# edwinb-ai/MolecularDynamics.jl

Hardware: AMD Instinct MI355X
Metric: particle-steps/sec + achieved HBM GB/s, 1M LJ particles rho=0.897, 1/2/4/8 GPUs (higher is better)
Workload: dtype f64; 1 GPU; BASELINE configs[2]: N=1048576 monodisperse LJ 3D rho=0.897 r_cut=2.5 dt=0.001 NVT Bussi tau=0.1 kT=1.4737, per GPU; particles_per_gpu=1048576, parallelism=1 GPU, step_loop=fused (k_step_tile: one launch per step + k_finalize), global_particles=1048576, tiled_force_kernel=True, max_tile_halo=2081, energies_every_step=False, thermo_frequency=2589

## Files before the change

include/mdhip.h:

```cpp
#ifndef MDHIP_H
#define MDHIP_H

#include <stdint.h>

#ifdef __cplusplus
extern "C" {
#endif

typedef struct md_ctx md_ctx;

enum { MD_POT_LJ = 0, MD_POT_PSEUDOHS = 1, MD_POT_POLYDISPERSE = 2, MD_POT_LJ_MODIFIED = 3, MD_POT_CUSTOM = 100 };

enum { MD_NVE = 0, MD_NVT = 1 };

int md_create(int dim, int64_t n_particles, const double *box, double list_cutoff, int device_id, md_ctx **out);
int md_destroy(md_ctx *ctx);

const char *md_last_error(md_ctx *ctx);

int md_set_potential(md_ctx *ctx, int kind, const double *params, int nparams);

int md_set_potential_source(md_ctx *ctx, const char *hip_src, const char *entry_name, const double *params,
                            int nparams);

// ... 65 lines not shown
                  const double *q, int nq);
int md_cage_origin(md_ctx *ctx, int slot);
int md_cage_sample(md_ctx *ctx, const int32_t *slots, const int32_t *rows, int count);
int md_cage_particles(md_ctx *ctx, int32_t *nnb, double *d2cr, int32_t *broken);
int md_cage_read(md_ctx *ctx, int64_t *nsamples, double *sums, int64_t *counts, int64_t *hist_broken, int64_t *overflow);
int md_cage_reset(md_ctx *ctx);

int md_kinetic(md_ctx *ctx, double *kinetic);

int md_scale_velocities(md_ctx *ctx, double s);

typedef struct {
    int64_t steps;
    int64_t rebuilds;
    int64_t violations;
    int64_t n_ghost;
    int64_t max_neighbors;
    double avg_neighbors;
    int64_t force_launches;
    double force_ms;
    int64_t max_halo;
    int64_t tiled;
    int64_t prunes;
    int64_t kickdrift_launches;
    double kickdrift_ms;
    int64_t fused;
    int64_t walked_outer;
    int64_t walked_inner;
    int64_t prune_launches_timed;
    double prune_ms;
    int64_t rebuilds_timed;
    double rebuild_ms;
    int64_t fused_build;
} md_stats;
int md_profile(md_ctx *ctx, int enable);
int md_get_stats(md_ctx *ctx, md_stats *out);

int md_create_domain(int dim, int64_t n_global, int64_t n_cap, const double *box, double list_cutoff,
                     int device_id, int rank, int nranks, md_ctx **out);
int md_dom_set_uniform(md_ctx *ctx, int uniform, double sigma);
int md_dom_upload(md_ctx *ctx, int64_t n_own, const int32_t *ids, const double *x, const double *v, const double *f,
                  const int32_t *images, const double *diameters);
int md_dom_download(md_ctx *ctx, int64_t cap, int64_t *n_own, int32_t *ids, double *x, double *v, double *f,
                    int32_t *images);
int md_dom_migrate_pack(md_ctx *ctx, int64_t *nsend );
int md_dom_migrate_unpack(md_ctx *ctx, const int64_t *nrecv );
int md_dom_halo_pack(md_ctx *ctx, int64_t *nsend );
int md_dom_halo_unpack(md_ctx *ctx, const int64_t *nrecv );
int md_dom_build(md_ctx *ctx);
int md_dom_set_step_buffers(md_ctx *ctx, void *send_left, void *send_right, void *recv_left, void *recv_right,
                            int64_t capacity_doubles);
int md_dom_get_sendbuf(md_ctx *ctx, int side, int64_t ndoubles, void *dst, int dst_is_device);
int md_dom_put_recvbuf(md_ctx *ctx, int side, int64_t ndoubles, const void *src, int src_is_device);
int md_dom_step_begin(md_ctx *ctx, double dt, int *violated);
int md_dom_step_end(md_ctx *ctx, double dt, int want_uw, double *uwk);
int md_dom_forces(md_ctx *ctx, double dt, int kick, int want_uw, double *uwk);
int md_dom_set_scale(md_ctx *ctx, double scale);
int md_dom_counts(md_ctx *ctx, int64_t *out );

int md_set_stream(md_ctx *ctx, void *hip_stream);
int md_dom_async_begin(md_ctx *ctx, int64_t nsteps, double dt, int ensemble, double tau, double nf, const double *ktemp,
                       const double *r1, const double *r2, int64_t prune_interval, void *flag_dev ,
                       void *kuw_dev );
int md_dom_step_a(md_ctx *ctx, double dt, int step);
int md_dom_step_b(md_ctx *ctx, double dt, int step, int want_uw);
int md_dom_step_c(md_ctx *ctx, int step, int want_uw);
// ... 19 lines not shown
```

moleculardynamics/jl_amd/_lib.py:

```python
import ctypes as C
import os

_HERE = os.path.dirname(os.path.abspath(__file__))
SO_PATH = os.path.join(_HERE, "csrc", "libmdhip.so")

MD_POT_LJ, MD_POT_PSEUDOHS, MD_POT_POLYDISPERSE, MD_POT_LJ_MODIFIED, MD_POT_CUSTOM = 0, 1, 2, 3, 100
MD_NVE, MD_NVT = 0, 1
MD_CLUSTER_ALL, MD_CLUSTER_SOLID = 0, 1

EXPORTS = [
    "md_create", "md_destroy", "md_last_error", "md_set_potential", "md_set_potential_source", "md_set_skin",
    "md_set_inner_skin",
    "md_upload", "md_download", "md_snapshot_begin", "md_snapshot_end", "md_compute_forces", "md_neighbor_pairs", "md_run", "md_kinetic",
    "md_scale_velocities", "md_profile", "md_get_stats", "md_version", "md_fire_minimize", "md_run_brownian",
    "md_create_domain", "md_dom_set_uniform", "md_dom_upload", "md_dom_download", "md_dom_migrate_pack",
    "md_dom_migrate_unpack", "md_dom_halo_pack", "md_dom_halo_unpack", "md_dom_build", "md_dom_get_sendbuf",
    "md_dom_put_recvbuf", "md_dom_set_step_buffers", "md_dom_step_begin", "md_dom_step_end", "md_dom_forces", "md_dom_set_scale",
    "md_dom_counts", "md_set_stream", "md_dom_async_begin", "md_dom_step_a", "md_dom_step_b", "md_dom_step_c",
    "md_dom_async_end", "md_dom_comm_unique_id", "md_dom_comm_init", "md_dom_run_window", "md_dom_rebuild",
    "md_dom_enable_pruning", "md_dom_max_disp0", "md_dom_invalidate_inner",
    "md_rdf_setup", "md_rdf_sample", "md_rdf_read", "md_rdf_reset",
    "md_dyn_setup", "md_dyn_origin", "md_dyn_sample", "md_dyn_read", "md_dyn_reset",
    "md_sq_setup", "md_sq_sample", "md_sq_rho", "md_sq_read", "md_sq_reset",
    "md_stress_setup", "md_stress_sample", "md_stress_tensor", "md_stress_read", "md_stress_reset",
    "md_boo_setup", "md_boo_sample", "md_boo_particles", "md_boo_qlm", "md_boo_read", "md_boo_reset",
    "md_cluster_setup", "md_cluster_sample", "md_cluster_particles", "md_cluster_read", "md_cluster_reset",
    "md_cage_setup", "md_cage_origin", "md_cage_sample", "md_cage_particles", "md_cage_read", "md_cage_reset",
]


class MdStats(C.Structure):
    _fields_ = [("steps", C.c_int64), ("rebuilds", C.c_int64), ("violations", C.c_int64), ("n_ghost", C.c_int64),
                ("max_neighbors", C.c_int64), ("avg_neighbors", C.c_double), ("force_launches", C.c_int64),
                ("force_ms", C.c_double), ("max_halo", C.c_int64), ("tiled", C.c_int64), ("prunes", C.c_int64),
                ("kickdrift_launches", C.c_int64), ("kickdrift_ms", C.c_double), ("fused", C.c_int64),
                ("walked_outer", C.c_int64), ("walked_inner", C.c_int64), ("prune_launches_timed", C.c_int64),
                ("prune_ms", C.c_double), ("rebuilds_timed", C.c_int64), ("rebuild_ms", C.c_double),
                ("fused_build", C.c_int64)]


class MdhipError(RuntimeError):
    pass


_lib = None


def load():
    global _lib
    if _lib is not None:
        return _lib
    if not os.path.exists(SO_PATH):
        raise MdhipError(
            f"{SO_PATH} not found: build it with `python -c 'import __graft_entry__ as g; g.build()'` or "
            "`make -C moleculardynamics/jl_amd/csrc`. There is no CPU fallback.")
    L = C.CDLL(SO_PATH)
    vp, dp, ip = C.c_void_p, C.POINTER(C.c_double), C.POINTER(C.c_int32)
    L.md_create.argtypes = [C.c_int, C.c_int64, dp, C.c_double, C.c_int, C.POINTER(vp)]
    L.md_create.restype = C.c_int
    L.md_destroy.argtypes = [vp]
    L.md_destroy.restype = C.c_int
    L.md_last_error.argtypes = [vp]
    L.md_last_error.restype = C.c_char_p
    L.md_set_potential.argtypes = [vp, C.c_int, dp, C.c_int]
    L.md_set_potential.restype = C.c_int
    L.md_set_potential_source.argtypes = [vp, C.c_char_p, C.c_char_p, dp, C.c_int]
    L.md_set_potential_source.restype = C.c_int
    L.md_set_skin.argtypes = [vp, C.c_double]
    L.md_set_skin.restype = C.c_int
    L.md_set_inner_skin.argtypes = [vp, C.c_double]
    L.md_set_inner_skin.restype = C.c_int
# ... 141 lines not shown
```

moleculardynamics/jl_amd/csrc/md_build_tile.hpp:

```cpp
#pragma once

#define MD_BT_THREADS 512
#define MD_SCAP 3584
#define MD_NCMAX 1024
#define MD_NEMAX 36
#define MD_INF_CELL 0x7fffffff
#define MD_SWB 8

#define MD_HALF_CELLS 14

typedef float md_f2 __attribute__((ext_vector_type(2)));

template <int D>
__device__ __forceinline__ unsigned tile_sweep_word(md_f2 xi2, md_f2 yi2, md_f2 zi2, md_f2 rl2, int qa, int qb,
                                                    const float *px, const float *py, const float *pz)
{
    unsigned w = ~0u;
    for (int q0 = qa; q0 < qb; q0 += 4) {
        float4 x4 = *(const float4 *)(px + q0);
        float4 y4 = *(const float4 *)(py + q0);
        md_f2 dxa = md_f2{x4.x, x4.y} - xi2, dxb = md_f2{x4.z, x4.w} - xi2;
        md_f2 dya = md_f2{y4.x, y4.y} - yi2, dyb = md_f2{y4.z, y4.w} - yi2;
        md_f2 da = dxa * dxa, db = dxb * dxb;
        da = __builtin_elementwise_fma(dya, dya, da);
        db = __builtin_elementwise_fma(dyb, dyb, db);
        if constexpr (D == 3) {
            float4 z4 = *(const float4 *)(pz + q0);
            md_f2 dza = md_f2{z4.x, z4.y} - zi2, dzb = md_f2{z4.z, z4.w} - zi2;
            da = __builtin_elementwise_fma(dza, dza, da);
            db = __builtin_elementwise_fma(dzb, dzb, db);
        }
        const md_f2 ta = rl2 - da, tb = rl2 - db;
        w = __builtin_amdgcn_alignbit(w, __float_as_uint(ta.x), 31);
        w = __builtin_amdgcn_alignbit(w, __float_as_uint(ta.y), 31);
        w = __builtin_amdgcn_alignbit(w, __float_as_uint(tb.x), 31);
        w = __builtin_amdgcn_alignbit(w, __float_as_uint(tb.y), 31);
// ... 14 lines not shown
        mask0[ci] = 0u;
        mask1[ci] = 0u;
        qstart[ci] = 0;
        int nbi = n0 + ci;
        if (nbi >= n1) continue;
        int lo = ctab_row[nbi];
        if (lo == 0xffff) continue;
        int qs = coff[lo], qe = coff[lo + 1];
        if (qe - qs > 64) {
            *too_big = true;
            continue;
        }
        qstart[ci] = qs;
        unsigned m0 = tile_sweep_word<D>(xi2, yi2, zi2, rl2, qs, min(qs + 32, qe), px, py, pz);
        unsigned m1 = tile_sweep_word<D>(xi2, yi2, zi2, rl2, qs + 32, qe, px, py, pz);
        const unsigned so = (unsigned)(self_q - qs);
        if (so < (unsigned)(qe - qs)) {
            if (so < 32u)
                m0 &= ~(1u << so);
            else
                m1 &= ~(1u << (so - 32u));
        }
        if (m0) atomicOr(&refmask[2 * lo], m0);
        if (m1) atomicOr(&refmask[2 * lo + 1], m1);
        mask0[ci] = m0;
        mask1[ci] = m1;
        cnt += __popc(m0) + __popc(m1);
    }
    return cnt;
}

#define MD_BBMAX 1024
#define MD_ROWPITCH 132
#define MD_BT_POOL 68864

template <bool GUARD>
__device__ __forceinline__ int tile_emit_word(unsigned m, int qb, const uint16_t *newidx, uint16_t *row,
                                              uint16_t *grow, int lane, int maxn, int cnt, int rs)
{
    while (m) {
        const int b1 = __ffs((int)m) - 1;
        const unsigned m1 = m & (m - 1u);
        const int b2 = __ffs((int)m1) - 1;
        m = m1 & (m1 - 1u);
        if (!GUARD || cnt + 1 < MD_ROWPITCH) {
            row[cnt] = (uint16_t)(qb + b1);
            if (m1) row[cnt + 1] = (uint16_t)(qb + b2);
        } else {
            if (cnt < MD_ROWPITCH)
                row[cnt] = (uint16_t)(qb + b1);
            else if (cnt < maxn)
                grow[row_off(cnt, lane)] = (uint16_t)((unsigned)newidx[qb + b1] * (unsigned)rs);
            if (m1 && cnt + 1 < maxn) grow[row_off(cnt + 1, lane)] = (uint16_t)((unsigned)newidx[qb + b2] * (unsigned)rs);
        }
        cnt += m1 ? 2 : 1;
    }
    return cnt;
}

template <bool GUARD>
__device__ __forceinline__ int tile_sweep_emit_lds(const unsigned *mask0, const unsigned *mask1, const int *qstart,
                                                   const uint16_t *newidx, uint16_t *row, uint16_t *grow, int lane,
                                                   int maxn, int cnt0, int rs)
{
    int cnt = cnt0;
#pragma unroll
    for (int ci = 0; ci < MD_HALF_CELLS; ++ci) {
        const int qs = qstart[ci];
        cnt = tile_emit_word<GUARD>(mask0[ci], qs, newidx, row, grow, lane, maxn, cnt, rs);
        cnt = tile_emit_word<GUARD>(mask1[ci], qs + 32, newidx, row, grow, lane, maxn, cnt, rs);
    }
    return cnt;
}


template <bool GUARD>
__device__ __forceinline__ int tile_compact_word(unsigned m, int base, int src0, uint16_t *newidx, uint32_t *hrow,
                                                 int hcap, int run)
{
    while (m) {
        const int bit = __ffs((int)m) - 1;
        m &= m - 1u;
        newidx[base + bit] = (uint16_t)run;
        if (!GUARD || run < hcap) hrow[run] = (uint32_t)(src0 + bit);
        ++run;
    }
    return run;
}

__device__ __forceinline__ float tile_staged_coord(float v) { return fabsf(v) < 1.0e29f ? v : 1.0e30f; }
__device__ __forceinline__ float tile_own_coord(float v) { return fabsf(v) < 1.0e29f ? v : -1.0e30f; }

template <int D>
__global__ void __launch_bounds__(MD_BT_THREADS)
    k_build_tile(int n, DevState s, BoxGrid g, float rl2f, const int32_t *__restrict__ cell_start,
                 const int32_t *__restrict__ cell_end, uint16_t *__restrict__ nlist16, int maxn,
                 int32_t *__restrict__ nneigh, int32_t *__restrict__ nmax_tile, uint32_t *__restrict__ halo, int hcap,
                 int32_t *__restrict__ halo_count, Scalars *sc, long long *__restrict__ stamps, int rs)
{
#define MD_STAMP(i)                                                                                   \
    do {                                                                                              \
        if (stamps && threadIdx.x == 0) stamps[(size_t)blockIdx.x * 10 + (i)] = (long long)clock64(); \
    } while (0)
    MD_STAMP(0);
    __shared__ __attribute__((aligned(16))) unsigned char pool[MD_BT_POOL];
    float *px = (float *)pool, *py = px + MD_SCAP, *pz = py + MD_SCAP;
    unsigned *refmask = (unsigned *)(pool + 43008);
    int *ucell = (int *)(pool + 51200);
    int *coff = (int *)(pool + 55296);
    int *lcell = (int *)(pool + 59408);
    uint16_t *ctab = (uint16_t *)(pool + 63504);
    uint16_t *lmap = (uint16_t *)(pool + 65552);
    uint16_t *blk2u = (uint16_t *)(pool + 67600);
    unsigned char *ccnt = (unsigned char *)(pool + 67840);
    __shared__ uint16_t newidx[MD_SCAP];
    __shared__ int cntA[MD_TILE], cntB[MD_TILE];
    __shared__ int sh_misc[16];
    __shared__ int sh_scan[16];
    __shared__ int sh_ne[MD_NEMAX];
    __shared__ int sh_ne_e[MD_NEMAX][3];

    const int tile = blockIdx.x;
    const int tid = threadIdx.x, lane = tid & 63;
    const int half = tid / MD_TILE;
    const int pt = tid - half * MD_TILE;
    const int k = tile * MD_TILE + pt;
    const bool active = k < n;
    const double4 *__restrict__ P = s.pos;
    const int NNB = (D == 3) ? 27 : 9;
    const int nA = (NNB + 1) / 2;

    const double4 org = P[tile * MD_TILE];
    double4 pd = P[active ? k : n - 1];
    const float xi = tile_own_coord((float)(pd.x - org.x)), yi = tile_own_coord((float)(pd.y - org.y)),
                zi = (D == 3) ? tile_own_coord((float)(pd.z - org.z)) : 0.f;
    int ec[3];
    cell_coords<D>(pd, g, ec);
#pragma unroll
    for (int c = 0; c < D; ++c) ec[c] += 1;
    const int mycell = ext_linear(ec, g);
    if (tid == 0) sh_misc[0] = mycell;
    const int last_active = min(n - 1, tile * MD_TILE + MD_TILE - 1) - tile * MD_TILE;
    if (tid == last_active) sh_misc[1] = mycell;
    if (tid == 0) {
        sh_misc[2] = 0;
        sh_misc[4] = sh_misc[5] = sh_misc[6] = 0x7fffffff;
        sh_misc[7] = sh_misc[8] = sh_misc[9] = -1;
// ... 120 lines not shown
    }
    int self_q = -1;
    if (active) {
        int uc = ctab[myci * NNB + (NNB >> 1)];
        self_q = coff[uc] + (k - cell_start[mycell]);
    }
    __syncthreads();
    MD_STAMP(4);
    const int wt = tile * (MD_TILE / 64) + (pt >> 6);
    const int n0 = half ? nA : 0, n1 = half ? NNB : nA;
    unsigned hmask0[MD_HALF_CELLS], hmask1[MD_HALF_CELLS];
    int qstart[MD_HALF_CELLS];
    int cnt = 0;
    bool too_big = false;
    if (active)
        cnt = tile_sweep_mark<D>(xi, yi, zi, ctab + myci * NNB, rl2f, self_q, n0, n1, px, py, pz, coff, refmask, hmask0,
                                 hmask1, qstart, &too_big);
    else {
#pragma unroll
        for (int ci = 0; ci < MD_HALF_CELLS; ++ci) {
            hmask0[ci] = hmask1[ci] = 0u;
            qstart[ci] = 0;
        }
    }
    if (too_big) atomicOr(&sc->halo_overflow, 4);
    if (half == 0)
        cntA[pt] = cnt;
    else
        cntB[pt] = cnt;
    __syncthreads();
    MD_STAMP(5);
    int H;
    {
        const int per = (MD_NCMAX + MD_BT_THREADS - 1) / MD_BT_THREADS;
        int c = 0;
        for (int q = 0; q < per; ++q) {
            int u = tid * per + q;
            if (u < nu) c += __popc(refmask[2 * u]) + __popc(refmask[2 * u + 1]);
        }
        int run = block_excl_scan(c, sh_scan, &H);
        uint32_t *hrow = halo + (size_t)tile * hcap;
        for (int q = 0; q < per; ++q) {
            int u = tid * per + q;
            if (u >= nu) continue;
            const int base = coff[u], src0 = cell_start[ucell[u]];
            const unsigned r0 = refmask[2 * u], r1 = refmask[2 * u + 1];
            if (run + __popc(r0) + __popc(r1) <= hcap) {
                run = tile_compact_word<false>(r0, base, src0, newidx, hrow, hcap, run);
                run = tile_compact_word<false>(r1, base + 32, src0 + 32, newidx, hrow, hcap, run);
            } else {
                run = tile_compact_word<true>(r0, base, src0, newidx, hrow, hcap, run);
                run = tile_compact_word<true>(r1, base + 32, src0 + 32, newidx, hrow, hcap, run);
            }
        }
        if (tid == 0) {
            halo_count[tile] = H;
            atomicMax(&sc->hmax, H);
            if (H > hcap || (H + 1) * rs > 65535) atomicOr(&sc->halo_overflow, 1);
        }
    }
    const int totp = cntA[pt] + cntB[pt];
    if (half == 0) {
        int tot = active ? totp : 0;
        if (active) {
            nneigh[k] = tot;
            if (tot > maxn) {
                atomicOr(&sc->overflow, 1);
                tot = maxn;
            }
        }
        int m = wave_max_i(tot);
        m = (m + 3) & ~3;
        if (m > maxn) m = maxn;
        if (lane == 0) {
            nmax_tile[wt] = m;
            sh_misc[10 + (pt >> 6)] = m;
        }
    }
    MD_STAMP(6);
// ... 49 lines not shown
```

moleculardynamics/jl_amd/csrc/md_kernels.hpp:

```cpp
#ifndef MD_RTC
#pragma once
#include <hip/hip_runtime.h>
#include <stdint.h>
#else
typedef __hip_internal::uint64_t uint64_t;
typedef __hip_internal::uint32_t uint32_t;
typedef __hip_internal::int32_t int32_t;
typedef __hip_internal::uint16_t uint16_t;
#endif

#define MD_BLOCK 256
#define MD_WAVE 64
#define MD_SENTINEL_POS 1.0e100
#define MD_VAL_SRC_BITS 26
#define MD_VAL_SRC_MASK ((1u << MD_VAL_SRC_BITS) - 1u)
#define MD_NO_VIOLATION 0x7fffffff

enum { POT_LJ = 0, POT_PSEUDOHS = 1, POT_POLYDISPERSE = 2, POT_LJ_MOD = 3, POT_CUSTOM = 100 };

struct DevState {
    double4 *pos;
    double *v[3];
    double *f[3];
    int32_t *img[3];
// ... 1231 lines not shown
    if constexpr (KICK) {
        double t = block_sum(ke, red);
        if (threadIdx.x == 0) partials[bid] = t;
    }
    if constexpr (WANT_UW) {
        double tu = block_sum(us, red);
        double tw = block_sum(ws, red);
        if (threadIdx.x == 0) {
            partials[nblk_total + bid] = tu;
            partials[2 * nblk_total + bid] = tw;
        }
    }
    MD_SSTAMP(5);
#undef MD_SSTAMP
}

struct StepBufs {
    const double2 *recA;
    double2 *recB;
    size_t rstride;
    const double *fA[3];
    double *fB[3];
    double4 *posB;
};

template <int D, int POT, bool UNIFORM, bool WANT_UW, bool PRUNE>
__global__ void __launch_bounds__(MD_TILE)
    k_step_tile(int n, DevState s, StepBufs sb, PotParams pp, const uint16_t *__restrict__ nlist16, int maxn,
                const int32_t *__restrict__ nmax_tile, const uint32_t *__restrict__ halo, int hcap,
                const int32_t *__restrict__ halo_count, double dt, double skin_half, double inner_half, int use_d1,
                double *__restrict__ partials, int nblk_total, Scalars *__restrict__ sc, int step,
                uint16_t *__restrict__ rows_in, int32_t *__restrict__ nmax_in, double rin2,
                long long *__restrict__ stamps, uint32_t *__restrict__ halo_in, int hcap_in,
                int32_t *__restrict__ halo_in_count, const int32_t *__restrict__ tile_list = nullptr)
{
#define MD_SSTAMP(i)                                                                                   \
    do {                                                                                               \
        if (stamps && (threadIdx.x & 63) == 0)                                                         \
            stamps[((size_t)blockIdx.x * 4 + (threadIdx.x >> 6)) * 8 + (i)] = (long long)clock64();   \
    } while (0)
    constexpr int RS = UNIFORM ? 24 : 32;
    extern __shared__ __attribute__((aligned(16))) unsigned char smem[];
    __shared__ double red[16];
    if (sc->first_viol < step) return;
    MD_SSTAMP(0);
    int bid = xcd_remap(blockIdx.x, gridDim.x);
    if (tile_list) bid = tile_list[bid];
    int H = halo_count[bid];
    const uint32_t *hl = halo + (size_t)bid * hcap;
    int k = bid * MD_TILE + threadIdx.x;
    bool active = k < n;
    int kk = active ? k : n - 1;
    int lane = threadIdx.x & 63;
    int wt = bid * (MD_TILE / 64) + (threadIdx.x >> 6);
    const ushort4 *row4 = (const ushort4 *)(nlist16 + ((size_t)wt * maxn) * 64) + lane;
    PruneRow rin64;
    rin64.base = PRUNE ? (unsigned char *)(rows_in + ((size_t)__builtin_amdgcn_readfirstlane(wt) * maxn) * 64) : nullptr;
    rin64.off = (unsigned)lane * 8u;
    unsigned long long acc = 0ull;
    int cin = 0;
    int m = nmax_tile[wt];
    const double alpha = sc->scale;
    const double adt = alpha * dt;
    const double2 *RA0 = sb.recA, *RA1 = RA0 + sb.rstride, *RA2 = RA1 + sb.rstride, *RA3 = RA2 + sb.rstride;
    double2 a0 = RA0[kk], a1 = RA1[kk], a2 = RA2[kk];
    double sig_own = pp.sig_u;
    if constexpr (!UNIFORM) sig_own = RA3[kk].x;
    double fprev[3] = {0.0, 0.0, 0.0}, xr[3] = {0.0, 0.0, 0.0};
#pragma unroll
    for (int c = 0; c < D; ++c) {
        fprev[c] = sb.fA[c][kk];
        xr[c] = PRUNE ? s.x0[c][kk] : s.x1[c][kk];
    }
    constexpr int G = MD_UNROLL / 4;
    ushort4 jn[G];
#pragma unroll
    for (int g = 0; g < G; ++g) jn[g] = row4[(size_t)((4 * g < m) ? g : 0) * 64];
    MD_SSTAMP(1);
#ifndef MD_STAGE_NB
#define MD_STAGE_NB ((!PRUNE && UNIFORM && !WANT_UW) ? 6 : 8)
#endif
    constexpr int NB = MD_STAGE_NB;
    for (int h0 = 0; h0 <= H; h0 += NB * MD_TILE) {
        uint32_t idx[NB];
#pragma unroll
        for (int i = 0; i < NB; ++i) {
            int h = h0 + i * MD_TILE + threadIdx.x;
            idx[i] = (h < H) ? hl[h] : 0xffffffffu;
        }
        double2 r0[NB], r1[NB], r2[NB], r3[NB];
#pragma unroll
        for (int i = 0; i < NB; ++i) {
            bool ok = idx[i] != 0xffffffffu;
            size_t j = ok ? (size_t)(idx[i] & 0x3ffffffu) : 0;
            r0[i] = RA0[j];
            r1[i] = RA1[j];
            r2[i] = RA2[j];
            if constexpr (!UNIFORM) r3[i] = RA3[j];
        }
#pragma unroll
        for (int i = 0; i < NB; ++i) {
            int h = h0 + i * MD_TILE + threadIdx.x;
            bool ok = idx[i] != 0xffffffffu;
            double x = __builtin_fma(adt, r1[i].y, r0[i].x);
            double y = __builtin_fma(adt, r2[i].x, r0[i].y);
            double z = (D == 3) ? __builtin_fma(adt, r2[i].y, r1[i].x) : 0.0;
            uint32_t code = ok ? (idx[i] >> 26) : 0u;
            if (code) shift_xyz(x, y, z, code, s.boxL, s.tric, s.cellA);
            if (!ok) {
                x = MD_SENTINEL_POS;
                y = MD_SENTINEL_POS;
                z = (D == 3) ? MD_SENTINEL_POS : 0.0;
            }
            if (h <= H) {
                double *rec = (double *)(smem + (size_t)h * RS);
                rec[0] = x;
                rec[1] = y;
                rec[2] = z;
                if constexpr (!UNIFORM) rec[3] = ok ? r3[i].x : 1.0;
            }
        }
    }
    const double pown[3] = {a0.x, a0.y, a1.x}, vown[3] = {a1.y, a2.x, a2.y};
    double vh[3] = {0.0, 0.0, 0.0}, xn[3] = {0.0, 0.0, 0.0};
    double disp2 = 0.0;
#pragma unroll
    for (int c = 0; c < D; ++c) {
        vh[c] = alpha * vown[c] + (fprev[c] * dt) / 2.0;
        xn[c] = __builtin_fma(adt, vown[c], pown[c]);
        double d = xn[c] - xr[c];
        disp2 = __builtin_fma(d, d, disp2);
    }
    const double4 pi = make_double4(xn[0], xn[1], xn[2], sig_own);
    if (active) sb.posB[k] = pi;
    {
        double d1 = use_d1 ? sqrt(__longlong_as_double((long long)sc->d1max2_bits)) : 0.0;
        double thr = fmin(inner_half, skin_half - d1);
        double thr2 = thr > 0.0 ? thr * thr : -1.0;
        if (__any(active && disp2 > thr2)) {
            if (lane == 0) atomicMin(&sc->first_viol, step);
        }
    }
    MD_SSTAMP(2);
    __syncthreads();
    MD_SSTAMP(3);
    double fx = 0.0, fy = 0.0, fz = 0.0, us = 0.0, ws = 0.0;
    tile_pair_loop<D, POT, UNIFORM, WANT_UW, PRUNE>(smem, row4, jn, m, H, pi, pp, rin64, rin2, acc, cin, fx, fy, fz, us, ws, nullptr);
    MD_SSTAMP(4);
    if constexpr (PRUNE) tile_prune_tail<D, UNIFORM>(s, sc, H, k, active, lane, wt, pi, rin64, nmax_in, acc, cin);
    double ke = 0.0;
    if (active) {
        const double fn[3] = {fx, fy, fz};
        const double h2 = (dt * dt) / 2.0;
        double vp[3] = {0.0, 0.0, 0.0}, pn[3] = {0.0, 0.0, 0.0};
#pragma unroll
        for (int c = 0; c < D; ++c) {
            sb.fB[c][k] = fn[c];
            vp[c] = vh[c] + (fn[c] * dt) / 2.0;
            pn[c] = __builtin_fma(h2, fn[c], xn[c]);
            ke += vp[c] * vp[c];
        }
        double2 *RB = sb.recB;
        RB[k] = make_double2(pn[0], pn[1]);
        RB[sb.rstride + k] = make_double2(pn[2], vp[0]);
        RB[2 * sb.rstride + k] = make_double2(vp[1], vp[2]);
        if constexpr (!UNIFORM) RB[3 * sb.rstride + k] = make_double2(sig_own, 0.0);
    } else {
// ... 483 lines not shown
```

moleculardynamics/jl_amd/csrc/mdhip.hip:

```cpp
#include <cstring>
#include <cstdlib>
#include <unistd.h>

#include "md_kernels.hpp"
#include "md_domain.hpp"
#include "md_rdf.hpp"
#include "md_dyn.hpp"
#include "md_sq.hpp"
#include "md_stress.hpp"
#include "md_boo.hpp"
#include "md_cluster.hpp"
#include "md_cage.hpp"

#include <rocprim/rocprim.hpp>

#include <algorithm>
#include <climits>
#include <cmath>
#include <cstdio>
#include <cstring>
#include <stdexcept>
#include <string>
#include <vector>

// ... 117 lines not shown
    double skin_req = 0.6;
    double skin = 0.0;
    double rl = 0.0;
    int pot_kind = POT_LJ;
    PotParams pp{};
    RtcModule *rtc = nullptr;
    bool uniform_sigma = true;
    double sigma_u = 1.0;
    double sigma_max = 1.0;
    int device = 0;
    hipStream_t stream = nullptr;
    hipStream_t own_stream = nullptr;

    int64_t cap = 0;
    int64_t next = 0;
    int64_t nghost = 0;
    StateBufs sb[2];
    int cur = 0;
    BoxGrid grid{};
    int ncell_ext = 0;

    DBuf<int32_t> nimg, img_off, newslot, gsrc, gowner, cell_start, cell_end, nneigh, nmax_tile;
    DBuf<uint32_t> gcode, vals_in, vals_out, nlist, halo;
    DBuf<uint16_t> nlist16;
    DBuf<int32_t> halo_count;
    DBuf<long long> dbg_stamps;
    int hcap = 4096;
    int hstride = 0;
    size_t tile_lds = 0;
    bool use_tiles = false;
    int tile_rs = 24;
    bool allow_tiles = true;
    bool allow_fused_build = true;
    bool have_nlist32 = false;
    DBuf<uint64_t> keys_in, keys_out;
    DBuf<char> sort_tmp, scan_tmp;
    int maxn = 0;
    int64_t ntiles = 0;

    DBuf<double> partials;
    DBuf<double> fire_part;
    DBuf<FireState> fire_state;
    DBuf<double> brown_acc;
    int nblk = 0;
    DBuf<Scalars> scal;
    DBuf<double> d_kt, d_r1, d_r2;

    DBuf<double> io_x, io_v, io_f, io_d;
    DBuf<int32_t> io_i;
    DBuf<double> snap_x;
    DBuf<int32_t> snap_i;
    double *pin_x = nullptr;
    int32_t *pin_i = nullptr;
    size_t pin_n = 0;
    hipStream_t copy_stream = nullptr;
    hipEvent_t ev_snap_ready = nullptr, ev_snap_copied = nullptr;
    bool snap_pending = false;

    bool list_valid = false;
    int64_t steps_since_build = 0;
    int64_t target_interval = 8;
    double inner_skin_req = 0.16;
    double inner_skin = 0.0;
    bool virtual_ghosts = false;
    bool inner_valid = false;
    bool prune_on = false;
// ... 454 lines not shown
    int64_t next = total;
    int n = (int)n_new;
    int32_t nghost = (int32_t)(next - n_new);
    if (nghost < 0) throw HipError("internal: fewer sort entries than owned particles");
    ensure_capacity(c, next);
    so = c->dev(c->cur);
    DevState sn = c->dev(c->cur ^ 1);

    k_emit<D><<<nbs, MD_BLOCK, 0, st>>>(n_src, n_own_src, so, g, alive, c->img_off.p, c->keys_in.p, c->vals_in.p,
                                        c->cell_start.p, c->cell_end.p, c->ncell_ext + 1);
    unsigned begin_bit = (unsigned)g.id_bits, end_bit = (unsigned)(g.id_bits + g.cell_bits + 1);
    tmp_bytes = 0;
    HIPCHK(rocprim::radix_sort_pairs(nullptr, tmp_bytes, c->keys_in.p, c->keys_out.p, c->vals_in.p, c->vals_out.p,
                                     (size_t)next, begin_bit, end_bit, st));
    c->sort_tmp.ensure(tmp_bytes);
    HIPCHK(rocprim::radix_sort_pairs(c->sort_tmp.p, tmp_bytes, c->keys_in.p, c->keys_out.p, c->vals_in.p,
                                     c->vals_out.p, (size_t)next, begin_bit, end_bit, st));
    k_gather<D><<<nblocks(next), MD_BLOCK, 0, st>>>(n, (int)next, so, sn, g, c->keys_out.p, c->vals_out.p,
                                                     c->newslot.p, c->gsrc.p, c->gcode.p, c->cell_start.p,
                                                     c->cell_end.p, c->scal.p);
    if (nghost > 0)
        k_ghost_owner<<<nblocks(nghost), MD_BLOCK, 0, st>>>(nghost, c->gsrc.p, c->newslot.p, c->gowner.p);
    c->cur ^= 1;
    c->next = next;
    c->nghost = nghost;
    c->n = n_new;
    c->nblk = nblocks(n_new);
    c->src_count = n_new;
    int nb = c->nblk;

    double rl2 = c->rl * c->rl;
    c->use_tiles = false;
    c->have_nlist32 = false;
    bool tile_ok = false;
    const int rs = (c->uniform_sigma && c->pot_kind != POT_POLYDISPERSE && c->pot_kind != POT_LJ_MOD && c->pot_kind != POT_CUSTOM) ? 24 : 32;
    auto set_tiles = [&](const Scalars &h) {
        size_t bytes = ((size_t)(h.hmax + 1) * rs + 15) & ~(size_t)15;
        if (!(h.halo_overflow) && bytes <= 150 * 1024) {
            c->use_tiles = true;
            c->hstride = h.hmax;
            c->tile_lds = bytes;
            c->tile_rs = rs;
            if (const char *e = getenv("MDHIP_LDS_PAD")) c->tile_lds += (size_t)atoi(e);
            return true;
        }
        return false;
    };
    auto grow_rows = [&]() {
        c->maxn = ((c->maxn * 3 / 2) + 3) & ~3;
        c->nlist.alloc((size_t)c->ntiles * c->maxn * 64);
        c->nlist16.alloc((size_t)c->ntiles * c->maxn * 64);
    };
    if (c->allow_tiles && c->allow_fused_build) {
        float rl2f = (float)(rl2 * (1.0 + 1.0e-4));
        for (int attempt = 0; attempt < 8; ++attempt) {
            if (attempt > 0 || next == 0) k_reset_flags<<<1, 1, 0, st>>>(c->scal.p);
            k_build_tile<D><<<c->nblk, MD_BT_THREADS, 0, st>>>(n, sn, g, rl2f, c->cell_start.p, c->cell_end.p,
                                                               c->nlist16.p, c->maxn, c->nneigh.p, c->nmax_tile.p,
                                                               c->halo.p, c->hcap, c->halo_count.p, c->scal.p,
                                                               c->dbg_stamps.p, rs);
            if (c->dbg_stamps.p) {
                std::vector<long long> hs((size_t)c->nblk * 10);
                HIPCHK(hipMemcpyAsync(hs.data(), c->dbg_stamps.p, hs.size() * 8, hipMemcpyDeviceToHost, st));
                HIPCHK(hipStreamSynchronize(st));
                double acc[9] = {0};
                for (int b = 0; b < c->nblk; ++b)
                    for (int i = 1; i <= 8; ++i) acc[i] += (double)(hs[(size_t)b * 10 + i] - hs[(size_t)b * 10 + i - 1]);
                fprintf(stderr, "[mdhip] build_tile phase cycles/block: cand %.0f sort %.0f uniq %.0f stage %.0f sweep0 %.0f compact %.0f sweep1 %.0f tail %.0f\n",
                        acc[1] / c->nblk, acc[2] / c->nblk, acc[3] / c->nblk, acc[4] / c->nblk, acc[5] / c->nblk,
                        acc[6] / c->nblk, acc[7] / c->nblk, acc[8] / c->nblk);
            }
            Scalars h;
            HIPCHK(hipMemcpyAsync(&h, c->scal.p, sizeof(Scalars), hipMemcpyDeviceToHost, st));
            HIPCHK(hipStreamSynchronize(st));
            if (getenv("MDHIP_DEBUG"))
                fprintf(stderr, "[mdhip] fused build: Rmax=%d Smax=%d Hmax=%d halo_overflow=%d row_overflow=%d maxn=%d\n",
                        h.dbg_rmax, h.dbg_smax, h.hmax, h.halo_overflow, h.overflow, c->maxn);
            if (h.halo_overflow) break;
            if (h.overflow) {
                grow_rows();
                continue;
            }
            tile_ok = set_tiles(h);
            break;
        }
    }
    if (!tile_ok) {
        for (int attempt = 0; attempt < 8; ++attempt) {
            k_reset_flags<<<1, 1, 0, st>>>(c->scal.p);
            k_build_list<D><<<nb, MD_BLOCK, 0, st>>>(n, sn, g, rl2, c->cell_start.p, c->cell_end.p, c->nlist.p,
                                                     c->maxn, c->nneigh.p, c->nmax_tile.p, (uint32_t)c->cap,
                                                     c->scal.p);
            Scalars h;
            HIPCHK(hipMemcpyAsync(&h, c->scal.p, sizeof(Scalars), hipMemcpyDeviceToHost, st));
            HIPCHK(hipStreamSynchronize(st));
            if (!h.overflow) break;
            if (attempt == 7) throw HipError("neighbour rows keep overflowing");
            grow_rows();
        }
        c->have_nlist32 = true;
        if (c->allow_tiles) {
            static int attr_dev_mask2 = 0;
            size_t lds = (size_t)MD_HT * 4 + (size_t)MD_HT * 2 + (MD_TILE + 1) * 4;
            if (!(attr_dev_mask2 & (1 << (c->device & 31)))) {
                HIPCHK(hipFuncSetAttribute((const void *)k_tile_localize, hipFuncAttributeMaxDynamicSharedMemorySize, (int)lds));
                attr_dev_mask2 |= 1 << (c->device & 31);
            }
            k_tile_localize<<<c->nblk, MD_TILE, lds, st>>>(c->nlist.p, c->nlist16.p, c->maxn, c->nmax_tile.p,
                                                           (uint32_t)c->cap, c->halo.p, c->hcap, c->halo_count.p,
                                                           c->scal.p, rs);
            Scalars h;
            HIPCHK(hipMemcpyAsync(&h, c->scal.p, sizeof(Scalars), hipMemcpyDeviceToHost, st));
            HIPCHK(hipStreamSynchronize(st));
            set_tiles(h);
        }
    }
// ... 377 lines not shown
            k_unfuse<2, true><<<c->nblk, MD_BLOCK, 0, c->stream>>>(n, s, rec, rec_stride(c), c->scal.p, ap);
        else
            k_unfuse<2, false><<<c->nblk, MD_BLOCK, 0, c->stream>>>(n, s, rec, rec_stride(c), c->scal.p, ap);
    }
    c->fz_a = 0;
}

template <int D, int POT, bool UNIFORM>
void launch_step_tpu(md_ctx *c, bool want_uw, double dt, int step)
{
    int n = (int)c->n;
    int nb = c->nblk;
    bool prune_step = c->prune_on && !c->inner_valid;
    bool use_inner = c->inner_valid;
    const uint16_t *rows16 = use_inner ? c->nlist16_in.p : c->nlist16.p;
    const int32_t *rowmax = use_inner ? c->nmax_tile_in.p : c->nmax_tile.p;
    double skin_half = 0.5 * c->skin;
    double inner_half = use_inner ? 0.5 * c->inner_skin : 0.5 * c->skin;
    int use_d1 = use_inner ? 1 : 0;
    DevState s = c->dev(c->cur);
    double rin = c->rc + c->inner_skin;
    const bool whole = c->part.list == nullptr;
    hipStream_t lst = whole ? c->stream : c->part.stream;
    const int grid = whole ? nb : c->part.count;
    if (prune_step) {
        for (int d = 0; d < 3; ++d) s.x1[d] = c->x1[d].p;
        if (whole) k_reset_d1<<<1, 1, 0, c->stream>>>(c->scal.p, step - 1);
    }
    const uint32_t *halo_p = c->halo.p;
    int halo_cap = c->hcap;
    const int32_t *halo_cnt = c->halo_count.p;
    size_t lds_bytes = c->tile_lds;
    uint32_t *hin_p = nullptr;
    if (prune_step) {
        c->inner_halo_live = false;
    } else if (use_inner && c->inner_halo_live) {
        halo_p = c->halo_in.p;
        halo_cap = c->hcap_in;
        halo_cnt = c->halo_in_count.p;
        lds_bytes = c->tile_lds_in;
    }
    const int a = c->fz_a;
    StateBufs &A = c->sb[c->cur ^ a], &B = c->sb[c->cur ^ a ^ 1];
    StepBufs sbufs{};
    sbufs.recA = c->rec[a].p;
    sbufs.recB = c->rec[a ^ 1].p;
    sbufs.rstride = rec_stride(c);
    for (int d = 0; d < 3; ++d) {
        sbufs.fA[d] = A.f[d].p;
        sbufs.fB[d] = B.f[d].p;
    }
    sbufs.posB = B.pos.p;
#define LS(UW, PR)                                                                                                  \
    do {                                                                                                            \
        auto kfn = k_step_tile<D, POT, UNIFORM, UW, PR>;                                                            \
        static int attr_dev_mask = 0;                                                                               \
        if (!(attr_dev_mask & (1 << (c->device & 31)))) {                                                           \
            HIPCHK(hipFuncSetAttribute((const void *)kfn, hipFuncAttributeMaxDynamicSharedMemorySize,               \
                                       (int)(160 * 1024 - 2048)));                                                  \
            attr_dev_mask |= 1 << (c->device & 31);                                                                 \
        }                                                                                                           \
        if (grid > 0)                                                                                               \
            kfn<<<grid, MD_TILE, lds_bytes, lst>>>(n, s, sbufs, c->pp, rows16, c->maxn, rowmax, halo_p, halo_cap,   \
                                                   halo_cnt, dt, skin_half, inner_half, use_d1,                     \
                                                   c->partials.p, nb, c->scal.p, step, c->nlist16_in.p,             \
                                                   c->nmax_tile_in.p, rin * rin, c->dbg_stamps.p, hin_p,            \
                                                   c->hcap_in, c->halo_in_count.p, c->part.list);                   \
    } while (0)
    if (whole) prof_begin(c, prune_step ? 3 : 0);
    if (prune_step) {
        if (want_uw)
            LS(true, true);
        else
            LS(false, true);
    } else {
        if (want_uw)
            LS(true, false);
        else
            LS(false, false);
    }
    if (whole) prof_end(c);
#undef LS
    if (!whole && !c->part.last) return;
    c->fz_a ^= 1;
    if (prune_step) {
        c->inner_valid = true;
        c->steps_since_prune = 0;
        c->st_prunes++;
    }
}

template <int D>
void launch_step_d(md_ctx *c, bool want_uw, double dt, int step)
{
    bool u = c->uniform_sigma;
    switch (c->pot_kind) {
    case POT_LJ:
        if (u)
            launch_step_tpu<D, POT_LJ, true>(c, want_uw, dt, step);
        else
// ... 332 lines not shown
        ctx->device = device_id;
        HIPCHK(hipSetDevice(device_id));
        if (domain) {
            int plo = 0, phi = 0;
            HIPCHK(hipDeviceGetStreamPriorityRange(&plo, &phi));
            HIPCHK(hipStreamCreateWithPriority(&ctx->stream, hipStreamNonBlocking, phi));
        } else {
            HIPCHK(hipStreamCreateWithFlags(&ctx->stream, hipStreamNonBlocking));
        }
        ctx->own_stream = ctx->stream;
        ctx->dim = dim;
        ctx->n_global = n_global;
        ctx->ncap = n_cap;
        ctx->n = domain ? 0 : n_cap;
        for (int c = 0; c < dim; ++c) ctx->L[c] = box[c * dim + c];
        ctx->tric = cg.tric;
        for (int c = 0; c < 9; ++c) {
            ctx->A[c] = cg.A[c];
            ctx->Ainv[c] = cg.Ainv[c];
        }
        for (int c = 0; c < 3; ++c) ctx->perp[c] = cg.perp[c];
        ctx->volume = cg.volume;
        ctx->rc = list_cutoff;
        if (domain) {
            ctx->dom.on = true;
            ctx->skin_req = 0.4;
            ctx->dom.rank = rank;
            ctx->dom.nranks = nranks;
            ctx->dom.xlo = ctx->L[0] * rank / nranks;
            ctx->dom.xhi = (rank == nranks - 1) ? ctx->L[0] : ctx->L[0] * (rank + 1) / nranks;
        }
        if (const char *e = getenv("MDHIP_NO_TILES")) ctx->allow_tiles = !(e[0] == '1');
        if (const char *e = getenv("MDHIP_NO_FUSED_BUILD")) ctx->allow_fused_build = !(e[0] == '1');
        if (const char *e = getenv("MDHIP_INNER_SKIN")) ctx->inner_skin_req = atof(e);
        if (const char *e = getenv("MDHIP_NO_FUSED_STEP")) ctx->allow_fused = !(e[0] == '1');
        ctx->allow_inner_halo = false;
        if (const char *e = getenv("MDHIP_INNER_HALO")) ctx->allow_inner_halo = (e[0] == '1');
        ctx->pot_kind = POT_LJ;
        ctx->pp.p[0] = 1.0;
        ctx->pp.p[1] = 1.0;
        ctx->pp.p[2] = 2.5;
        configure_grid(ctx);
        configure_potential(ctx);
        double frac = 1.0;
        for (int c = 0; c < dim; ++c) frac *= (double)ctx->grid.ncx[c] / ctx->grid.nc[c];
        int64_t gcap = (int64_t)((frac - 1.0) * 1.3 * n_cap) + 4096;
        ctx->cap = n_cap + gcap;
        alloc_state(ctx, 0, ctx->cap);
        alloc_state(ctx, 1, ctx->cap);
        int64_t n = n_cap;
        ctx->nimg.alloc(ctx->cap + 2);
        ctx->img_off.alloc(ctx->cap + 2);
        HIPCHK(hipMemsetAsync(ctx->nimg.p, 0, sizeof(int32_t) * (ctx->cap + 2), ctx->stream));
        ctx->newslot.alloc(ctx->cap + 1);
        ctx->keys_in.alloc(ctx->cap);
        ctx->keys_out.alloc(ctx->cap);
        ctx->vals_in.alloc(ctx->cap);
        ctx->vals_out.alloc(ctx->cap);
        ctx->gsrc.alloc(ctx->cap + 1);
        ctx->gcode.alloc(ctx->cap + 1);
        ctx->gowner.alloc(ctx->cap + 1);
        ctx->nblk = nblocks(ctx->n);
        int nblk_cap = nblocks(n);
        ctx->ntiles = (int64_t)nblk_cap * (MD_BLOCK / 64);
        ctx->nneigh.alloc(n);
        ctx->nmax_tile.alloc(ctx->ntiles);
// ... 1891 lines not shown
        std::vector<int32_t> h((size_t)ctx->n);
        HIPCHK(hipMemcpyAsync(h.data(), ctx->nneigh.p, sizeof(int32_t) * ctx->n, hipMemcpyDeviceToHost, ctx->stream));
        HIPCHK(hipStreamSynchronize(ctx->stream));
        double sum = 0.0;
        for (int32_t v : h) sum += v;
        out->avg_neighbors = sum / (double)ctx->n;
    }
    out->prunes = ctx->st_prunes;
    out->max_halo = ctx->use_tiles ? ctx->hstride : 0;
    out->tiled = ctx->use_tiles ? 1 : 0;
    out->force_launches = ctx->prof_launch_acc;
    out->force_ms = ctx->prof_ms_acc;
    out->kickdrift_launches = ctx->prof_kd_launch_acc;
    out->kickdrift_ms = ctx->prof_kd_ms_acc;
    out->fused = ctx->last_run_fused ? 1 : 0;
    out->walked_outer = out->walked_inner = 0;
    if (ctx->list_valid) {
        const int64_t nw = (ctx->n + 63) / 64;
        std::vector<int32_t> h((size_t)nw);
        HIPCHK(hipMemcpyAsync(h.data(), ctx->nmax_tile.p, sizeof(int32_t) * nw, hipMemcpyDeviceToHost, ctx->stream));
        HIPCHK(hipStreamSynchronize(ctx->stream));
        for (int32_t v : h) out->walked_outer += 64 * (int64_t)v;
        if (ctx->inner_valid) {
            HIPCHK(hipMemcpyAsync(h.data(), ctx->nmax_tile_in.p, sizeof(int32_t) * nw, hipMemcpyDeviceToHost, ctx->stream));
            HIPCHK(hipStreamSynchronize(ctx->stream));
            for (int32_t v : h) out->walked_inner += 64 * (int64_t)v;
        }
    }
    out->prune_launches_timed = ctx->prof_prune_acc;
    out->prune_ms = ctx->prof_prune_ms_acc;
    out->rebuilds_timed = ctx->prof_rebuild_acc;
    out->rebuild_ms = ctx->prof_rebuild_ms_acc;
    out->fused_build = (ctx->list_valid && ctx->use_tiles && !ctx->have_nlist32) ? 1 : 0;
    API_END
}


namespace {
void dom_require(md_ctx *c)
{
    if (!c->dom.on) throw HipError("this handle was not created with md_create_domain");
}
DomCounters dom_read_counters(md_ctx *c)
{
    DomCounters h;
    HIPCHK(hipMemcpyAsync(&h, c->dom.counters.p, sizeof h, hipMemcpyDeviceToHost, c->stream));
    HIPCHK(hipStreamSynchronize(c->stream));
    if (h.error & 1) throw HipError("a particle moved by more than one slab between list builds");
    if (h.error & 2) throw HipError("slab exchange buffer overflow (raise n_cap)");
    return h;
}
}

int md_dom_set_uniform(md_ctx *ctx, int uniform, double sigma)
{
    API_BEGIN
    dom_require(ctx);
    ctx->uniform_sigma = uniform != 0;
    ctx->sigma_u = sigma;
    configure_potential(ctx);
    ctx->list_valid = false;
    API_END
}

int md_dom_upload(md_ctx *ctx, int64_t n_own, const int32_t *ids, const double *x, const double *v, const double *f,
                  const int32_t *images, const double *diameters)
// ... 1312 lines not shown
```

Before: 6.767 billion particle-steps/s.

## Place tile-owned particles first in halo and stage them from registers

```diff
diff --git a/include/mdhip.h b/include/mdhip.h
--- a/include/mdhip.h
+++ b/include/mdhip.h
@@ -121,6 +121,7 @@
     int64_t rebuilds_timed;
     double rebuild_ms;
     int64_t fused_build;
+    int64_t own_first;
 } md_stats;
 int md_profile(md_ctx *ctx, int enable);
 int md_get_stats(md_ctx *ctx, md_stats *out);
diff --git a/moleculardynamics/jl_amd/_lib.py b/moleculardynamics/jl_amd/_lib.py
--- a/moleculardynamics/jl_amd/_lib.py
+++ b/moleculardynamics/jl_amd/_lib.py
@@ -36,7 +36,7 @@
                 ("kickdrift_launches", C.c_int64), ("kickdrift_ms", C.c_double), ("fused", C.c_int64),
                 ("walked_outer", C.c_int64), ("walked_inner", C.c_int64), ("prune_launches_timed", C.c_int64),
                 ("prune_ms", C.c_double), ("rebuilds_timed", C.c_int64), ("rebuild_ms", C.c_double),
-                ("fused_build", C.c_int64)]
+                ("fused_build", C.c_int64), ("own_first", C.c_int64)]
 
 
 class MdhipError(RuntimeError):
diff --git a/moleculardynamics/jl_amd/csrc/md_build_tile.hpp b/moleculardynamics/jl_amd/csrc/md_build_tile.hpp
--- a/moleculardynamics/jl_amd/csrc/md_build_tile.hpp
+++ b/moleculardynamics/jl_amd/csrc/md_build_tile.hpp
@@ -1,7 +1,7 @@
 #pragma once
 
 #define MD_BT_THREADS 512
-#define MD_SCAP 3584
+#define MD_SCAP 4096
 #define MD_NCMAX 1024
 #define MD_NEMAX 36
 #define MD_INF_CELL 0x7fffffff
@@ -82,7 +82,7 @@
 
 #define MD_BBMAX 1024
 #define MD_ROWPITCH 132
-#define MD_BT_POOL 68864
+#define MD_BT_POOL 68880
 
 template <bool GUARD>
 __device__ __forceinline__ int tile_emit_word(unsigned m, int qb, const uint16_t *newidx, uint16_t *row,
@@ -146,7 +146,7 @@
     k_build_tile(int n, DevState s, BoxGrid g, float rl2f, const int32_t *__restrict__ cell_start,
                  const int32_t *__restrict__ cell_end, uint16_t *__restrict__ nlist16, int maxn,
                  int32_t *__restrict__ nneigh, int32_t *__restrict__ nmax_tile, uint32_t *__restrict__ halo, int hcap,
-                 int32_t *__restrict__ halo_count, Scalars *sc, long long *__restrict__ stamps, int rs)
+                 int32_t *__restrict__ halo_count, Scalars *sc, long long *__restrict__ stamps, int rs, int own_first)
 {
 #define MD_STAMP(i)                                                                                   \
     do {                                                                                              \
@@ -155,14 +155,17 @@
     MD_STAMP(0);
     __shared__ __attribute__((aligned(16))) unsigned char pool[MD_BT_POOL];
     float *px = (float *)pool, *py = px + MD_SCAP, *pz = py + MD_SCAP;
-    unsigned *refmask = (unsigned *)(pool + 43008);
-    int *ucell = (int *)(pool + 51200);
-    int *coff = (int *)(pool + 55296);
-    int *lcell = (int *)(pool + 59408);
-    uint16_t *ctab = (uint16_t *)(pool + 63504);
-    uint16_t *lmap = (uint16_t *)(pool + 65552);
+    int *lcell = (int *)(pool + 43008);
+    uint16_t *lmap = (uint16_t *)(pool + 47104);
+    unsigned *refmask = (unsigned *)(pool + 49152);
+    int *ucell = (int *)(pool + 57344);
+    int *coff = (int *)(pool + 61440);
+    uint16_t *ctab = (uint16_t *)(pool + 65552);
     uint16_t *blk2u = (uint16_t *)(pool + 67600);
-    unsigned char *ccnt = (unsigned char *)(pool + 67840);
+    unsigned char *ccnt = (unsigned char *)(pool + 67856);
+    static_assert(3 * MD_SCAP * 4 == 49152 && MD_BBMAX * 6 == 49152 - 43008 && 67856 + MD_NCMAX == MD_BT_POOL &&
+                      MD_BT_POOL >= MD_TILE * MD_ROWPITCH * 2,
+                  "LDS layout of k_build_tile");
     __shared__ uint16_t newidx[MD_SCAP];
     __shared__ int cntA[MD_TILE], cntB[MD_TILE];
     __shared__ int sh_misc[16];
@@ -349,19 +352,41 @@
     MD_STAMP(5);
     int H;
     {
-        const int per = (MD_NCMAX + MD_BT_THREADS - 1) / MD_BT_THREADS;
+        const int hown = own_first ? MD_TILE : 0;
+        const int own0 = tile * MD_TILE, own1 = own_first ? min(n, own0 + MD_TILE) : own0;
+        constexpr int per = (MD_NCMAX + MD_BT_THREADS - 1) / MD_BT_THREADS;
+        unsigned rm0[per], rm1[per];
+        int csrc[per];
         int c = 0;
+#pragma unroll
         for (int q = 0; q < per; ++q) {
             int u = tid * per + q;
-            if (u < nu) c += __popc(refmask[2 * u]) + __popc(refmask[2 * u + 1]);
-        }
-        int run = block_excl_scan(c, sh_scan, &H);
+            rm0[q] = rm1[q] = 0u;
+            csrc[q] = 0;
+            if (u < nu) {
+                const int src0 = cell_start[ucell[u]];
+                const int lo = max(own0 - src0, 0), hi = min(own1 - src0, 64);
+                unsigned long long r = ((unsigned long long)refmask[2 * u + 1] << 32) | refmask[2 * u];
+                if (hi > lo) r &= ~((~0ull >> (64 - (hi - lo))) << lo);
+                rm0[q] = (unsigned)r;
+                rm1[q] = (unsigned)(r >> 32);
+                csrc[q] = src0;
+                c += __popcll(r);
+            }
+        }
+        int run = hown + block_excl_scan(c, sh_scan, &H);
+        H += hown;
         uint32_t *hrow = halo + (size_t)tile * hcap;
+        if (own_first && half == 0) {
+            if (active) newidx[self_q] = (uint16_t)pt;
+            if (pt < hcap) hrow[pt] = (uint32_t)(active ? k : own0);
+        }
+#pragma unroll
         for (int q = 0; q < per; ++q) {
             int u = tid * per + q;
             if (u >= nu) continue;
-            const int base = coff[u], src0 = cell_start[ucell[u]];
-            const unsigned r0 = refmask[2 * u], r1 = refmask[2 * u + 1];
+            const int base = coff[u], src0 = csrc[q];
+            const unsigned r0 = rm0[q], r1 = rm1[q];
             if (run + __popc(r0) + __popc(r1) <= hcap) {
                 run = tile_compact_word<false>(r0, base, src0, newidx, hrow, hcap, run);
                 run = tile_compact_word<false>(r1, base + 32, src0 + 32, newidx, hrow, hcap, run);
diff --git a/moleculardynamics/jl_amd/csrc/md_kernels.hpp b/moleculardynamics/jl_amd/csrc/md_kernels.hpp
--- a/moleculardynamics/jl_amd/csrc/md_kernels.hpp
+++ b/moleculardynamics/jl_amd/csrc/md_kernels.hpp
@@ -1287,7 +1287,7 @@
                 double *__restrict__ partials, int nblk_total, Scalars *__restrict__ sc, int step,
                 uint16_t *__restrict__ rows_in, int32_t *__restrict__ nmax_in, double rin2,
                 long long *__restrict__ stamps, uint32_t *__restrict__ halo_in, int hcap_in,
-                int32_t *__restrict__ halo_in_count, const int32_t *__restrict__ tile_list = nullptr)
+                int32_t *__restrict__ halo_in_count, int own_first, const int32_t *__restrict__ tile_list = nullptr)
 {
 #define MD_SSTAMP(i)                                                                                   \
     do {                                                                                               \
@@ -1336,45 +1336,48 @@
 #define MD_STAGE_NB ((!PRUNE && UNIFORM && !WANT_UW) ? 6 : 8)
 #endif
     constexpr int NB = MD_STAGE_NB;
-    for (int h0 = 0; h0 <= H; h0 += NB * MD_TILE) {
+    const unsigned char *hlb = (const unsigned char *)hl;
+    const unsigned char *PA0 = (const unsigned char *)RA0, *PA1 = (const unsigned char *)RA1,
+                        *PA2 = (const unsigned char *)RA2, *PA3 = (const unsigned char *)RA3;
+    for (int h0 = own_first ? MD_TILE : 0; h0 < H; h0 += NB * MD_TILE) {
         uint32_t idx[NB];
 #pragma unroll
         for (int i = 0; i < NB; ++i) {
             int h = h0 + i * MD_TILE + threadIdx.x;
-            idx[i] = (h < H) ? hl[h] : 0xffffffffu;
+            idx[i] = *(const uint32_t *)(hlb + (uint32_t)min(h, H - 1) * 4u);
         }
         double2 r0[NB], r1[NB], r2[NB], r3[NB];
 #pragma unroll
         for (int i = 0; i < NB; ++i) {
-            bool ok = idx[i] != 0xffffffffu;
-            size_t j = ok ? (size_t)(idx[i] & 0x3ffffffu) : 0;
-            r0[i] = RA0[j];
-            r1[i] = RA1[j];
-            r2[i] = RA2[j];
-            if constexpr (!UNIFORM) r3[i] = RA3[j];
+            const uint32_t jo = (idx[i] & 0x3ffffffu) * 16u;
+            r0[i] = *(const double2 *)(PA0 + jo);
+            r1[i] = *(const double2 *)(PA1 + jo);
+            r2[i] = *(const double2 *)(PA2 + jo);
+            if constexpr (!UNIFORM) r3[i] = *(const double2 *)(PA3 + jo);
         }
 #pragma unroll
         for (int i = 0; i < NB; ++i) {
             int h = h0 + i * MD_TILE + threadIdx.x;
-            bool ok = idx[i] != 0xffffffffu;
             double x = __builtin_fma(adt, r1[i].y, r0[i].x);
             double y = __builtin_fma(adt, r2[i].x, r0[i].y);
             double z = (D == 3) ? __builtin_fma(adt, r2[i].y, r1[i].x) : 0.0;
-            uint32_t code = ok ? (idx[i] >> 26) : 0u;
+            uint32_t code = idx[i] >> 26;
             if (code) shift_xyz(x, y, z, code, s.boxL, s.tric, s.cellA);
-            if (!ok) {
-                x = MD_SENTINEL_POS;
-                y = MD_SENTINEL_POS;
-                z = (D == 3) ? MD_SENTINEL_POS : 0.0;
-            }
-            if (h <= H) {
+            if (h < H) {
                 double *rec = (double *)(smem + (size_t)h * RS);
                 rec[0] = x;
                 rec[1] = y;
                 rec[2] = z;
-                if constexpr (!UNIFORM) rec[3] = ok ? r3[i].x : 1.0;
+                if constexpr (!UNIFORM) rec[3] = r3[i].x;
             }
         }
+    }
+    if (threadIdx.x == 0) {
+        double *rec = (double *)(smem + (size_t)H * RS);
+        rec[0] = MD_SENTINEL_POS;
+        rec[1] = MD_SENTINEL_POS;
+        rec[2] = (D == 3) ? MD_SENTINEL_POS : 0.0;
+        if constexpr (!UNIFORM) rec[3] = 1.0;
     }
     const double pown[3] = {a0.x, a0.y, a1.x}, vown[3] = {a1.y, a2.x, a2.y};
     double vh[3] = {0.0, 0.0, 0.0}, xn[3] = {0.0, 0.0, 0.0};
@@ -1388,6 +1391,13 @@
     }
     const double4 pi = make_double4(xn[0], xn[1], xn[2], sig_own);
     if (active) sb.posB[k] = pi;
+    if (own_first) {
+        double *rec = (double *)(smem + (size_t)threadIdx.x * RS);
+        rec[0] = active ? xn[0] : MD_SENTINEL_POS;
+        rec[1] = active ? xn[1] : MD_SENTINEL_POS;
+        rec[2] = (active || D != 3) ? xn[2] : MD_SENTINEL_POS;
+        if constexpr (!UNIFORM) rec[3] = active ? sig_own : 1.0;
+    }
     {
         double d1 = use_d1 ? sqrt(__longlong_as_double((long long)sc->d1max2_bits)) : 0.0;
         double thr = fmin(inner_half, skin_half - d1);
diff --git a/moleculardynamics/jl_amd/csrc/mdhip.hip b/moleculardynamics/jl_amd/csrc/mdhip.hip
--- a/moleculardynamics/jl_amd/csrc/mdhip.hip
+++ b/moleculardynamics/jl_amd/csrc/mdhip.hip
@@ -173,6 +173,9 @@
     int tile_rs = 24;
     bool allow_tiles = true;
     bool allow_fused_build = true;
+    bool allow_own_first = true;
+    bool own_first = false;
+    bool own_first_staged = false;
     bool have_nlist32 = false;
     DBuf<uint64_t> keys_in, keys_out;
     DBuf<char> sort_tmp, scan_tmp;
@@ -693,6 +696,7 @@
     double rl2 = c->rl * c->rl;
     c->use_tiles = false;
     c->have_nlist32 = false;
+    c->own_first = false;
     bool tile_ok = false;
     const int rs = (c->uniform_sigma && c->pot_kind != POT_POLYDISPERSE && c->pot_kind != POT_LJ_MOD && c->pot_kind != POT_CUSTOM) ? 24 : 32;
     auto set_tiles = [&](const Scalars &h) {
@@ -719,7 +723,7 @@
             k_build_tile<D><<<c->nblk, MD_BT_THREADS, 0, st>>>(n, sn, g, rl2f, c->cell_start.p, c->cell_end.p,
                                                                c->nlist16.p, c->maxn, c->nneigh.p, c->nmax_tile.p,
                                                                c->halo.p, c->hcap, c->halo_count.p, c->scal.p,
-                                                               c->dbg_stamps.p, rs);
+                                                               c->dbg_stamps.p, rs, c->allow_own_first ? 1 : 0);
             if (c->dbg_stamps.p) {
                 std::vector<long long> hs((size_t)c->nblk * 10);
                 HIPCHK(hipMemcpyAsync(hs.data(), c->dbg_stamps.p, hs.size() * 8, hipMemcpyDeviceToHost, st));
@@ -743,6 +747,7 @@
                 continue;
             }
             tile_ok = set_tiles(h);
+            c->own_first = tile_ok && c->allow_own_first;
             break;
         }
     }
@@ -1186,6 +1191,7 @@
     const int32_t *halo_cnt = c->halo_count.p;
     size_t lds_bytes = c->tile_lds;
     uint32_t *hin_p = nullptr;
+    int own_first = c->own_first ? 1 : 0;
     if (prune_step) {
         c->inner_halo_live = false;
     } else if (use_inner && c->inner_halo_live) {
@@ -1193,7 +1199,9 @@
         halo_cap = c->hcap_in;
         halo_cnt = c->halo_in_count.p;
         lds_bytes = c->tile_lds_in;
-    }
+        own_first = 0;
+    }
+    c->own_first_staged = own_first != 0;
     const int a = c->fz_a;
     StateBufs &A = c->sb[c->cur ^ a], &B = c->sb[c->cur ^ a ^ 1];
     StepBufs sbufs{};
@@ -1219,7 +1227,7 @@
                                                    halo_cnt, dt, skin_half, inner_half, use_d1,                     \
                                                    c->partials.p, nb, c->scal.p, step, c->nlist16_in.p,             \
                                                    c->nmax_tile_in.p, rin * rin, c->dbg_stamps.p, hin_p,            \
-                                                   c->hcap_in, c->halo_in_count.p, c->part.list);                   \
+                                                   c->hcap_in, c->halo_in_count.p, own_first, c->part.list);        \
     } while (0)
     if (whole) prof_begin(c, prune_step ? 3 : 0);
     if (prune_step) {
@@ -1618,6 +1626,7 @@
         }
         if (const char *e = getenv("MDHIP_NO_TILES")) ctx->allow_tiles = !(e[0] == '1');
         if (const char *e = getenv("MDHIP_NO_FUSED_BUILD")) ctx->allow_fused_build = !(e[0] == '1');
+        if (const char *e = getenv("MDHIP_NO_OWN_FIRST")) ctx->allow_own_first = !(e[0] == '1');
         if (const char *e = getenv("MDHIP_INNER_SKIN")) ctx->inner_skin_req = atof(e);
         if (const char *e = getenv("MDHIP_NO_FUSED_STEP")) ctx->allow_fused = !(e[0] == '1');
         ctx->allow_inner_halo = false;
@@ -3575,6 +3584,7 @@
     out->rebuilds_timed = ctx->prof_rebuild_acc;
     out->rebuild_ms = ctx->prof_rebuild_ms_acc;
     out->fused_build = (ctx->list_valid && ctx->use_tiles && !ctx->have_nlist32) ? 1 : 0;
+    out->own_first = ctx->own_first_staged ? 1 : 0;
     API_END
 }
 
```

Measured after the change: 6.988 billion particle-steps/s (median of 6 runs). 3.3% higher.
